# AHupuJR/REFID

Measured on AMD Instinct MI355X. Metric: interpolated frames/sec (train step) GoPro 256x256 11+1, higher is better.
Workload: dtype f32

## Files before the change

refid_amd/csrc/conv_pw.hip:

```cpp
#include "common.h"
#include "conv_args.h"
#include <cstdlib>

namespace {

typedef unsigned int u32x4 __attribute__((ext_vector_type(4)));
typedef __bf16 bf16x8 __attribute__((ext_vector_type(8)));
constexpr int KC = 8;
__device__ constexpr int PW_TA[6] = {0, 1, 0, 2, 0, 1};
__device__ constexpr int PW_TB[6] = {0, 0, 1, 0, 2, 1};

__device__ __forceinline__ void pw_split8(const f32x4& v0, const f32x4& v1, f32x4 (&pl)[3]) {
    bf16x8 p0, p1, p2;
#pragma unroll
    for (int k = 0; k < 8; ++k) {
        const float v = k < 4 ? v0[k] : v1[k - 4];
        const __bf16 h = (__bf16)v;
        p0[k] = h;
        const float r = v - (float)h;
        const __bf16 m = (__bf16)r;
        p1[k] = m;
        p2[k] = (__bf16)(r - (float)m);
    }
    pl[0] = __builtin_bit_cast(f32x4, p0);
    pl[1] = __builtin_bit_cast(f32x4, p1);
    pl[2] = __builtin_bit_cast(f32x4, p2);
}
constexpr int OOB = -1;

__device__ __forceinline__ float gelu_erf(float x) { return 0.5f * x * (1.f + erff(x * 0.70710678118654752440f)); }
__device__ __forceinline__ float gelu_erf_d(float x) {
    const float cdf = 0.5f * (1.f + erff(x * 0.70710678118654752440f));
    const float pdf = 0.39894228040143267794f * __expf(-0.5f * x * x);
    return cdf + x * pdf;
}

template <int NT, int XD, bool EX, bool SIX = false>
__global__ __launch_bounds__(256, (SIX || NT > 2) ? 3 : 4) void conv_pw_kernel(const ConvKArgs a, const PwExtra e) {
    const int lane = threadIdx.x & 63, wave = threadIdx.x >> 6;
    const int li = lane & 31, kh = lane >> 5;
    const long long npix = (long long)a.N * a.H * a.W;
    const long long p0 = ((long long)blockIdx.x * 4 + wave) * 32;
    const long long p = p0 + li;
    const int n0 = blockIdx.y * (32 * NT);

    const long long spanA = a.patchW ? (npix / a.patchW) * (long long)a.patchRow : npix * a.ldA;
    const long long spanB = a.patchW ? spanA - a.patchRow / 2 : npix * (a.inB ? a.ldB : a.ldA);
    const __amdgpu_buffer_rsrc_t rsA = __builtin_amdgcn_make_buffer_rsrc(
        const_cast<float*>(a.inA), 0, (int)min(spanA * 4, 0x7fffffffLL), 0x00020000);
    const __amdgpu_buffer_rsrc_t rsB = __builtin_amdgcn_make_buffer_rsrc(
        const_cast<float*>(a.inB ? a.inB : a.inA), 0, (int)min(spanB * 4, 0x7fffffffLL), 0x00020000);
    const __amdgpu_buffer_rsrc_t rsW = __builtin_amdgcn_make_buffer_rsrc(
        const_cast<float*>(a.w), 0, (int)min((long long)a.nchunks * a.CoutPad * KC * (SIX ? 6 : 4), 0x7fffffffLL), 0x00020000);
    const bool pok = p < npix;
    const long long pA = a.patchW ? (p / a.patchW) * a.patchRow + (p % a.patchW) * a.ldA : p * a.ldA;
    const long long pB = a.patchW ? (p / a.patchW) * a.patchRow + (p % a.patchW) * a.ldB : p * a.ldB;
    const int voA = pok ? (int)(pA * 4) + kh * 16 : OOB;
    const int voB = pok ? (int)(pB * 4) + kh * 16 : OOB;
    int voW[NT];
#pragma unroll
    for (int nt = 0; nt < NT; ++nt) {
        const int row = a.coBase + n0 + nt * 32 + li;
        voW[nt] = (row < a.CoutPad) ? (SIX ? row * 32 + kh * 16 : (row * KC + kh * 4) * 4) : OOB;
    }
    const int wChunk = a.CoutPad * KC * 4;
    const int wPlane = a.CoutPad * 32;

    f32x16 acc[NT];
#pragma unroll
    for (int nt = 0; nt < NT; ++nt)
#pragma unroll
        for (int r = 0; r < 16; ++r) acc[nt][r] = 0.f;

    auto load_x = [&](int ch) -> f32x4 {
        const int c0 = ch * KC;
        const bool fromA = c0 < a.Ca;
        const int soff = (fromA ? c0 : c0 - a.Ca) * 4;
        const int vo = (c0 + kh * 4 < a.Ctot) ? (fromA ? voA : voB) : OOB;
        const u32x4 v = fromA ? __builtin_amdgcn_raw_buffer_load_b128(rsA, vo, soff, 0)
                              : __builtin_amdgcn_raw_buffer_load_b128(rsB, vo, soff, 0);
        return __builtin_bit_cast(f32x4, v);
    };
    auto load_w = [&](int ch, f32x4 (&dst)[NT]) {
#pragma unroll
        for (int nt = 0; nt < NT; ++nt)
            dst[nt] = __builtin_bit_cast(f32x4, __builtin_amdgcn_raw_buffer_load_b128(rsW, voW[nt], ch * wChunk, 0));
    };
    auto load_w6 = [&](int c16, f32x4 (&dst)[3][NT]) {
#pragma unroll
        for (int pl = 0; pl < 3; ++pl)
#pragma unroll
            for (int nt = 0; nt < NT; ++nt)
                dst[pl][nt] = __builtin_bit_cast(f32x4, __builtin_amdgcn_raw_buffer_load_b128(rsW, voW[nt], (c16 * 3 + pl) * wPlane, 0));
    };
    auto mfma6 = [&](const f32x4& x0, const f32x4& x1, const f32x4 (&w6)[3][NT]) {
        f32x4 pl[3];
        pw_split8(x0, x1, pl);
#pragma unroll
        for (int t = 0; t < 6; ++t)
#pragma unroll
            for (int nt = 0; nt < NT; ++nt)
                acc[nt] = __builtin_amdgcn_mfma_f32_32x32x16_bf16(__builtin_bit_cast(bf16x8, w6[PW_TA[t]][nt]),
                                                                  __builtin_bit_cast(bf16x8, pl[PW_TB[t]]), acc[nt], 0, 0, 0);
    };

    f32x4 xr[2 * XD];
    f32x4 wr[SIX ? 1 : 2][NT];
    f32x4 w6[SIX ? 2 : 1][3][NT];
    const int nch = a.nchunks;
    __shared__ float sS[EX ? 128 : 1];
    bool ln_done = false;
    if constexpr (EX) {
        if (e.pool != nullptr) {
            __shared__ float sM[128], sZ[64];
            const int C = e.seC, Ch = C / 2, tid = threadIdx.x;
            const int n = (int)(((long long)blockIdx.x * 128) / e.hw);
            for (int c = tid; c < C; c += 256) {
                const float* pp = e.pool + (long long)n * e.poolParts * C + c;
                float s0 = 0.f;
                for (int r = 0; r < e.poolParts; ++r) s0 += pp[(long long)r * C];
                sM[c] = s0 * e.invHW;
            }
            __syncthreads();
            for (int j = tid; j < Ch; j += 256) {
                float z = e.seB1[j];
                for (int c = 0; c < C; ++c) z += e.seW1[j * C + c] * sM[c];
                sZ[j] = z > 0.f ? z : 0.f;
            }
            __syncthreads();
            for (int c = tid; c < C; c += 256) {
                float v = e.seB2[c];
                for (int j = 0; j < Ch; ++j) v += e.seW2[c * Ch + j] * sZ[j];
                sS[c] = 1.f / (1.f + __expf(-v));
            }
            __syncthreads();
            if (e.seS != nullptr && blockIdx.y == 0 && ((long long)blockIdx.x * 128) % e.hw == 0) {
                for (int c = tid; c < C; c += 256) { e.seM[n * C + c] = sM[c]; e.seS[n * C + c] = sS[c]; }
                for (int j = tid; j < Ch; j += 256) e.seZ1[n * Ch + j] = sZ[j];
            }
        }
        if (e.lnG != nullptr) {
#pragma unroll
            for (int j = 0; j < 2 * XD; ++j) xr[j] = (j < nch) ? load_x(j) : f32x4{0.f, 0.f, 0.f, 0.f};
            if constexpr (SIX) load_w6(0, w6[0]);
            else load_w(0, wr[0]);
            float s1 = 0.f;
#pragma unroll
            for (int j = 0; j < 2 * XD; ++j) s1 += (xr[j][0] + xr[j][1]) + (xr[j][2] + xr[j][3]);
            s1 += __shfl_xor(s1, 32, 64);
            const float mu = s1 / (float)a.Ctot;
            float s2 = 0.f;
#pragma unroll
            for (int j = 0; j < 2 * XD; ++j)
                if (j < nch) {
#pragma unroll
                    for (int k = 0; k < 4; ++k) { const float d = xr[j][k] - mu; s2 += d * d; }
                }
            s2 += __shfl_xor(s2, 32, 64);
            const float rstd = 1.f / sqrtf(s2 / (float)a.Ctot + e.lnEps);
#pragma unroll
            for (int j = 0; j < 2 * XD; ++j)
                if (j < nch) {
                    const int c = j * KC + kh * 4;
                    const f32x4 gv = *reinterpret_cast<const f32x4*>(e.lnG + c);
                    const f32x4 bv = *reinterpret_cast<const f32x4*>(e.lnB + c);
#pragma unroll
                    for (int k = 0; k < 4; ++k) xr[j][k] = (xr[j][k] - mu) * rstd * gv[k] + bv[k];
                    if (e.lnOut != nullptr && blockIdx.y == 0 && pok)
                        *reinterpret_cast<f32x4*>(e.lnOut + p * e.ldLn + c) = xr[j];
                }
            if constexpr (SIX) {
#pragma unroll
                for (int j = 0; j < 2 * XD; j += 2)
                    if (j < nch) {
                        if (j + 2 < nch) load_w6(j / 2 + 1, w6[(j / 2 + 1) & 1]);
                        mfma6(xr[j], xr[j + 1], w6[(j / 2) & 1]);
                    }
            } else {
#pragma unroll
                for (int j = 0; j < 2 * XD; ++j)
                    if (j < nch) {
                        if (j + 1 < nch) load_w(j + 1, wr[(j + 1) & 1]);
#pragma unroll
                        for (int kk = 0; kk < 4; ++kk)
#pragma unroll
                            for (int nt = 0; nt < NT; ++nt)
                                acc[nt] = __builtin_amdgcn_mfma_f32_32x32x2f32(wr[j & 1][nt][kk], xr[j][kk], acc[nt], 0, 0, 0);
                    }
            }
            ln_done = true;
        }
    }
    if (!ln_done) {
#pragma unroll
        for (int j = 0; j < XD; ++j)
            if (j < nch) xr[j] = load_x(j);
        if constexpr (SIX) load_w6(0, w6[0]);
        else load_w(0, wr[0]);
        for (int c0 = 0; c0 < nch; c0 += 2 * XD) {
#pragma unroll
            for (int j = 0; j < 2 * XD; ++j) {
                const int c = c0 + j;
                if (c < nch) {
                    if constexpr (SIX) {
                        if ((j & 1) == 0 && c + 2 < nch) load_w6(c / 2 + 1, w6[(j / 2 + 1) & 1]);
                    } else {
                        if (c + 1 < nch) load_w(c + 1, wr[(j + 1) & 1]);
                    }
                    if (c + XD < nch) xr[(j + XD) % (2 * XD)] = load_x(c + XD);
                    if constexpr (EX) {
                        if (e.pool != nullptr) {
                            const int k0 = c * KC + kh * 4;
                            const f32x4 sv = *reinterpret_cast<const f32x4*>(&sS[k0 % e.seC]);
                            xr[j] *= sv;
                            if (e.xsOut != nullptr && blockIdx.y == 0 && pok)
                                *reinterpret_cast<f32x4*>(e.xsOut + p * e.ldXs + k0) = xr[j];
                        }
                    }
                    if constexpr (SIX) {
                        if (j & 1) mfma6(xr[j - 1], xr[j], w6[(j / 2) & 1]);
                    } else {
#pragma unroll
                        for (int kk = 0; kk < 4; ++kk)
#pragma unroll
                            for (int nt = 0; nt < NT; ++nt)
                                acc[nt] = __builtin_amdgcn_mfma_f32_32x32x2f32(wr[j & 1][nt][kk], xr[j][kk], acc[nt], 0, 0, 0);
                    }
                }
            }
        }
    }

    if (a.vecOK) {
        constexpr int HN = (NT > 2) ? 2 : NT;
        constexpr int PITCH = 8 * HN + 1;
        __shared__ f32x4 sT[4][32 * PITCH];
        f32x4* t = sT[wave];
#pragma unroll
        for (int h0 = 0; h0 < NT; h0 += HN) {
            if (h0) __syncthreads();
#pragma unroll
            for (int nt = 0; nt < HN; ++nt)
#pragma unroll
                for (int g = 0; g < 4; ++g) {
                    f32x4 v;
#pragma unroll
                    for (int k = 0; k < 4; ++k) v[k] = acc[h0 + nt][4 * g + k];
                    t[li * PITCH + nt * 8 + 2 * g + kh] = v;
                }
            __syncthreads();
#pragma unroll
            for (int it = 0; it < 4 * HN; ++it) {
                const int f = it * 64 + lane;
                const int px = f / (8 * HN), c4 = f % (8 * HN);
                const long long pp = p0 + px;
                const int j0 = n0 + h0 * 32 + c4 * 4;
                if (pp >= npix || j0 >= a.Cout) continue;
                f32x4 v = t[px * PITCH + c4];
                if (a.shuffle) {
                    const int Co1 = a.Cout >> 2;
                    const unsigned qd = (unsigned)j0 / (unsigned)Co1, ch = (unsigned)j0 - qd * Co1;
                    const unsigned up = (unsigned)pp, row = up / (unsigned)a.W, x = up - row * a.W;
                    const long long op = (long long)(2 * row + (qd >> 1)) * (2 * a.W) + 2 * x + (qd & 1);
                    if (a.bias) v += *reinterpret_cast<const f32x4*>(a.bias + ch);
                    lrelu4(v, a.slopePre, a.slopePre != 1.f);
                    if (a.res) v += *reinterpret_cast<const f32x4*>(a.res + op * a.ldR + ch);
                    lrelu4(v, a.slopePost, a.slopePost != 1.f);
                    *reinterpret_cast<f32x4*>(a.out + op * a.ldO + ch) = v;
                    continue;
                }
                if (a.bias) v += *reinterpret_cast<const f32x4*>(a.bias + a.coBase + j0);
                lrelu4(v, a.slopePre, a.slopePre != 1.f);
                if (a.res) v += *reinterpret_cast<const f32x4*>(a.res + pp * a.ldR + j0);
                if constexpr (EX) {
                    if (e.res2) v += *reinterpret_cast<const f32x4*>(e.res2 + pp * e.ldR2 + j0);
                }
                lrelu4(v, a.slopePost, a.slopePost != 1.f);
                if (a.mask) {
                    const f32x4 mv = *reinterpret_cast<const f32x4*>(a.mask + pp * a.ldM + j0);
                    if (a.maskMode == 1) {
#pragma unroll
                        for (int k = 0; k < 4; ++k) v[k] *= gelu_erf_d(mv[k]);
                    } else {
#pragma unroll
                        for (int k = 0; k < 4; ++k) v[k] *= (mv[k] > 0.f) ? 1.f : a.slopeMask;
                    }
                }
                *reinterpret_cast<f32x4*>(a.out + pp * a.ldO + j0) = v;
                if (a.out2)
                    *reinterpret_cast<f32x4*>(a.out2 + pp * a.ldO2 + j0) = v + *reinterpret_cast<const f32x4*>(a.add2 + pp * a.ldA2 + j0);
                if constexpr (EX) {
                    if (e.out2) {
                        f32x4 gl;
#pragma unroll
                        for (int k = 0; k < 4; ++k) gl[k] = gelu_erf(v[k]);
                        *reinterpret_cast<f32x4*>(e.out2 + pp * e.ldO2 + j0) = gl;
                    }
                }
            }
        }
        return;
    }
    if (!pok) return;
#pragma unroll
    for (int nt = 0; nt < NT; ++nt) {
#pragma unroll
        for (int g = 0; g < 4; ++g) {
            const int j0 = n0 + nt * 32 + 8 * g + 4 * kh;
#pragma unroll
            for (int k = 0; k < 4; ++k) {
                if (j0 + k >= a.Cout) break;
                float tv = acc[nt][4 * g + k] + (a.bias ? a.bias[a.coBase + j0 + k] : 0.f);
                tv = lrelu(tv, a.slopePre);
                if (a.res) tv += a.res[p * a.ldR + j0 + k];
                tv = lrelu(tv, a.slopePost);
                if (a.mask) tv *= a.maskMode == 1 ? gelu_erf_d(a.mask[p * a.ldM + j0 + k]) : ((a.mask[p * a.ldM + j0 + k] > 0.f) ? 1.f : a.slopeMask);
                a.out[p * a.ldO + j0 + k] = tv;
            }
        }
    }
}

}

int refid_launch_pointwise(const ConvKArgs& ka, hipStream_t st, const PwExtra* ex, int terms) {
    ConvKArgs a = ka;
    a.nchunks = cdiv(a.Ctot, KC);
    const long long npix = (long long)a.N * a.H * a.W;
    const int nb = (int)((npix + 127) / 128);
    const bool six = terms == 6;
    REFID_CHECK(!a.shuffle || (a.vecOK && ex == nullptr && terms == 0 && a.mask == nullptr && a.Cout > 32 && (a.Cout / 4) % 4 == 0 &&
                               npix < 0x7fffffffLL),
                "conv2d: ConvTranspose2d on the pointwise tile needs 16-byte aligned tensors, fp32 products, no mask / fusions and "
                "at least 16 output channels");
    REFID_CHECK(a.out2 == nullptr || (a.vecOK && ex == nullptr), "conv2d: the pointwise tile's second output needs 16-byte aligned tensors and no fusions");
    REFID_CHECK(!a.patchW || (terms == 0 && ex == nullptr && a.inB != nullptr), "conv2d: the patch form of the pointwise tile has fp32 products, no fusions");
    REFID_CHECK(terms == 0 || terms == 6, "conv2d: the pointwise tile has fp32 products (0) or six bf16 products (6), got %d", terms);
    REFID_CHECK(!six || (a.Ctot % 16 == 0 && (a.inB == nullptr || a.Ca % 16 == 0) && a.Cout > 32),
                "conv2d: the six-product pointwise tile needs channel counts that are multiples of 16 and more than 32 outputs");
    if (ex != nullptr) {
        REFID_CHECK(a.vecOK && a.Cout > 32, "conv2d: pointwise fusions need 16-byte aligned tensors and more than 32 outputs");
        REFID_CHECK(!ex->lnG || (a.inB == nullptr && a.Ctot % 8 == 0 && a.Ctot <= 64 && ex->lnB),
                    "conv2d: the LayerNorm prologue needs one source of at most 64 channels (got %d)", a.Ctot);
        REFID_CHECK(!ex->pool || (ex->hw > 0 && ex->hw % 128 == 0 && ex->seC >= 8 && ex->seC <= 128 && ex->seC % 8 == 0 &&
                                  a.Ctot % ex->seC == 0 && ex->poolParts > 0 && ex->seW1 && ex->seB1 && ex->seW2 && ex->seB2 &&
                                  (!ex->seS || (ex->seM && ex->seZ1)) && !ex->lnG),
                    "conv2d: bad squeeze-excite fusion arguments (pixels per sample must be a multiple of 128)");
        if (six) hipLaunchKernelGGL((conv_pw_kernel<2, 4, true, true>), dim3(nb, cdiv(a.Cout, 64)), dim3(256), 0, st, a, *ex);
        else hipLaunchKernelGGL((conv_pw_kernel<2, 4, true>), dim3(nb, cdiv(a.Cout, 64)), dim3(256), 0, st, a, *ex);
        REFID_LAUNCH_CHECK("conv_pw/fused");
        return 0;
    }
    const PwExtra none;
    if (six) hipLaunchKernelGGL((conv_pw_kernel<2, 4, false, true>), dim3(nb, cdiv(a.Cout, 64)), dim3(256), 0, st, a, none);
    else if (a.Cout <= 32) hipLaunchKernelGGL((conv_pw_kernel<1, 8, false>), dim3(nb, 1), dim3(256), 0, st, a, none);
    else {
        static const bool nt4 = []() { const char* e = getenv("REFID_PW_NT4"); return e && e[0] == '1'; }();
        if (nt4 && a.Cout % 128 == 0)
            hipLaunchKernelGGL((conv_pw_kernel<4, 4, false>), dim3(nb, a.Cout / 128), dim3(256), 0, st, a, none);
        else
            hipLaunchKernelGGL((conv_pw_kernel<2, 4, false>), dim3(nb, cdiv(a.Cout, 64)), dim3(256), 0, st, a, none);
    }
    REFID_LAUNCH_CHECK("conv_pw");
    return 0;
}
```

Before: 526.9.

## Software-pipeline pointwise conv main loop and epilogue with buffer loads

Adds a fast main-loop path for channel counts divisible by the unroll group. It uses a deeper weight register ring (for NT==1) and prefetches activations XD chunks ahead, with sched barriers and out-of-bounds buffer loads replacing bounds checks. The LayerNorm prologue gets a fully unrolled specialization with buffer stores, and the SE scaling is folded into the fast loop. The vectorized epilogue now prefetches residual, mask and second-residual tiles through buffer resources ahead of use, and has a dedicated pixel-shuffle path. The aim is to hide global memory latency behind MFMA work and epilogue math, at the cost of more registers and more code complexity.

```diff
diff --git a/refid_amd/csrc/conv_pw.hip b/refid_amd/csrc/conv_pw.hip
--- a/refid_amd/csrc/conv_pw.hip
+++ b/refid_amd/csrc/conv_pw.hip
@@ -1,6 +1,7 @@
 #include "common.h"
 #include "conv_args.h"
 #include <cstdlib>
+#include <type_traits>
 
 namespace {
 
@@ -40,7 +41,7 @@
     const int lane = threadIdx.x & 63, wave = threadIdx.x >> 6;
     const int li = lane & 31, kh = lane >> 5;
     const long long npix = (long long)a.N * a.H * a.W;
-    const long long p0 = ((long long)blockIdx.x * 4 + wave) * 32;
+    const long long p0 = ((long long)blockIdx.x * 4 + __builtin_amdgcn_readfirstlane(wave)) * 32;
     const long long p = p0 + li;
     const int n0 = blockIdx.y * (32 * NT);
 
@@ -86,12 +87,28 @@
         for (int nt = 0; nt < NT; ++nt)
             dst[nt] = __builtin_bit_cast(f32x4, __builtin_amdgcn_raw_buffer_load_b128(rsW, voW[nt], ch * wChunk, 0));
     };
+    auto load_w_sel = [&](int ch, f32x4 (&dst)[NT]) {
+        const bool ok = ch < a.nchunks;
+        const int so = ok ? ch * wChunk : 0;
+#pragma unroll
+        for (int nt = 0; nt < NT; ++nt)
+            dst[nt] = __builtin_bit_cast(f32x4, __builtin_amdgcn_raw_buffer_load_b128(rsW, ok ? voW[nt] : OOB, so, 0));
+    };
     auto load_w6 = [&](int c16, f32x4 (&dst)[3][NT]) {
 #pragma unroll
         for (int pl = 0; pl < 3; ++pl)
 #pragma unroll
             for (int nt = 0; nt < NT; ++nt)
                 dst[pl][nt] = __builtin_bit_cast(f32x4, __builtin_amdgcn_raw_buffer_load_b128(rsW, voW[nt], (c16 * 3 + pl) * wPlane, 0));
+    };
+    auto load_w6_sel = [&](int c16, f32x4 (&dst)[3][NT]) {
+        const bool ok = 2 * c16 < a.nchunks;
+#pragma unroll
+        for (int pl = 0; pl < 3; ++pl)
+#pragma unroll
+            for (int nt = 0; nt < NT; ++nt)
+                dst[pl][nt] = __builtin_bit_cast(f32x4, __builtin_amdgcn_raw_buffer_load_b128(rsW, ok ? voW[nt] : OOB,
+                                                                                              ok ? (c16 * 3 + pl) * wPlane : 0, 0));
     };
     auto mfma6 = [&](const f32x4& x0, const f32x4& x1, const f32x4 (&w6)[3][NT]) {
         f32x4 pl[3];
@@ -104,8 +121,10 @@
                                                                   __builtin_bit_cast(bf16x8, pl[PW_TB[t]]), acc[nt], 0, 0, 0);
     };
 
+    constexpr int WD = (NT == 1) ? 3 : 1;
+    static_assert((2 * XD) % (WD + 1) == 0, "the weight ring must divide the unrolled group");
     f32x4 xr[2 * XD];
-    f32x4 wr[SIX ? 1 : 2][NT];
+    f32x4 wr[SIX ? 1 : WD + 1][NT];
     f32x4 w6[SIX ? 2 : 1][3][NT];
     const int nch = a.nchunks;
     __shared__ float sS[EX ? 128 : 1];
@@ -140,58 +159,136 @@
             }
         }
         if (e.lnG != nullptr) {
-#pragma unroll
-            for (int j = 0; j < 2 * XD; ++j) xr[j] = (j < nch) ? load_x(j) : f32x4{0.f, 0.f, 0.f, 0.f};
+            const __amdgpu_buffer_rsrc_t rsLn = __builtin_amdgcn_make_buffer_rsrc(
+                e.lnOut + p0 * e.ldLn, 0, (e.lnOut != nullptr && blockIdx.y == 0) ? 0x7fffffff : 0, 0x00020000);
+            auto ln_body = [&](auto full_tag) {
+                constexpr bool FULL = decltype(full_tag)::value;
+#pragma unroll
+                for (int j = 0; j < 2 * XD; ++j) xr[j] = (FULL || j < nch) ? load_x(j) : f32x4{0.f, 0.f, 0.f, 0.f};
+                if constexpr (SIX) load_w6(0, w6[0]);
+                else load_w(0, wr[0]);
+                float s1 = 0.f;
+#pragma unroll
+                for (int j = 0; j < 2 * XD; ++j) s1 += (xr[j][0] + xr[j][1]) + (xr[j][2] + xr[j][3]);
+                s1 += __shfl_xor(s1, 32, 64);
+                const float mu = s1 / (float)a.Ctot;
+                float s2 = 0.f;
+#pragma unroll
+                for (int j = 0; j < 2 * XD; ++j)
+                    if (FULL || j < nch) {
+#pragma unroll
+                        for (int k = 0; k < 4; ++k) { const float d = xr[j][k] - mu; s2 += d * d; }
+                    }
+                s2 += __shfl_xor(s2, 32, 64);
+                const float rstd = 1.f / sqrtf(s2 / (float)a.Ctot + e.lnEps);
+#pragma unroll
+                for (int j = 0; j < 2 * XD; ++j)
+                    if (FULL || j < nch) {
+                        const int c = j * KC + kh * 4;
+                        const f32x4 gv = *reinterpret_cast<const f32x4*>(e.lnG + c);
+                        const f32x4 bv = *reinterpret_cast<const f32x4*>(e.lnB + c);
+#pragma unroll
+                        for (int k = 0; k < 4; ++k) xr[j][k] = (xr[j][k] - mu) * rstd * gv[k] + bv[k];
+                        if constexpr (FULL)
+                            __builtin_amdgcn_raw_buffer_store_b128(__builtin_bit_cast(u32x4, xr[j]), rsLn,
+                                                                   pok ? (li * e.ldLn + c) * 4 : OOB, 0, 0);
+                        else if (e.lnOut != nullptr && blockIdx.y == 0 && pok)
+                            *reinterpret_cast<f32x4*>(e.lnOut + p * e.ldLn + c) = xr[j];
+                    }
+                if constexpr (SIX) {
+#pragma unroll
+                    for (int j = 0; j < 2 * XD; j += 2)
+                        if (FULL || j < nch) {
+                            if constexpr (FULL) {
+                                if (j + 2 < 2 * XD) load_w6(j / 2 + 1, w6[(j / 2 + 1) & 1]);
+                                __builtin_amdgcn_sched_barrier(0);
+                            } else {
+                                if (j + 2 < nch) load_w6(j / 2 + 1, w6[(j / 2 + 1) & 1]);
+                            }
+                            mfma6(xr[j], xr[j + 1], w6[(j / 2) & 1]);
+                        }
+                } else {
+#pragma unroll
+                    for (int j = 0; j < 2 * XD; ++j)
+                        if (FULL || j < nch) {
+                            if constexpr (FULL) {
+                                if (j + 1 < 2 * XD) load_w(j + 1, wr[(j + 1) & 1]);
+                                __builtin_amdgcn_sched_barrier(0);
+                            } else {
+                                if (j + 1 < nch) load_w(j + 1, wr[(j + 1) & 1]);
+                            }
+#pragma unroll
+                            for (int kk = 0; kk < 4; ++kk)
+#pragma unroll
+                                for (int nt = 0; nt < NT; ++nt)
+                                    acc[nt] = __builtin_amdgcn_mfma_f32_32x32x2f32(wr[j & 1][nt][kk], xr[j][kk], acc[nt], 0, 0, 0);
+                        }
+                }
+            };
+            if (nch == 2 * XD) ln_body(std::true_type{});
+            else ln_body(std::false_type{});
+            ln_done = true;
+        }
+    }
+    if (!ln_done && nch % (2 * XD) == 0) {
+        auto k_fast = [&](auto se_tag) {
+            constexpr bool SE = decltype(se_tag)::value;
+            __amdgpu_buffer_rsrc_t rsXs = rsA;
+            if constexpr (SE)
+                rsXs = __builtin_amdgcn_make_buffer_rsrc(e.xsOut + p0 * e.ldXs, 0,
+                                                         (e.xsOut != nullptr && blockIdx.y == 0) ? 0x7fffffff : 0, 0x00020000);
             if constexpr (SIX) load_w6(0, w6[0]);
-            else load_w(0, wr[0]);
-            float s1 = 0.f;
-#pragma unroll
-            for (int j = 0; j < 2 * XD; ++j) s1 += (xr[j][0] + xr[j][1]) + (xr[j][2] + xr[j][3]);
-            s1 += __shfl_xor(s1, 32, 64);
-            const float mu = s1 / (float)a.Ctot;
-            float s2 = 0.f;
-#pragma unroll
-            for (int j = 0; j < 2 * XD; ++j)
-                if (j < nch) {
-#pragma unroll
-                    for (int k = 0; k < 4; ++k) { const float d = xr[j][k] - mu; s2 += d * d; }
-                }
-            s2 += __shfl_xor(s2, 32, 64);
-            const float rstd = 1.f / sqrtf(s2 / (float)a.Ctot + e.lnEps);
-#pragma unroll
-            for (int j = 0; j < 2 * XD; ++j)
-                if (j < nch) {
-                    const int c = j * KC + kh * 4;
-                    const f32x4 gv = *reinterpret_cast<const f32x4*>(e.lnG + c);
-                    const f32x4 bv = *reinterpret_cast<const f32x4*>(e.lnB + c);
-#pragma unroll
-                    for (int k = 0; k < 4; ++k) xr[j][k] = (xr[j][k] - mu) * rstd * gv[k] + bv[k];
-                    if (e.lnOut != nullptr && blockIdx.y == 0 && pok)
-                        *reinterpret_cast<f32x4*>(e.lnOut + p * e.ldLn + c) = xr[j];
-                }
-            if constexpr (SIX) {
-#pragma unroll
-                for (int j = 0; j < 2 * XD; j += 2)
-                    if (j < nch) {
-                        if (j + 2 < nch) load_w6(j / 2 + 1, w6[(j / 2 + 1) & 1]);
-                        mfma6(xr[j], xr[j + 1], w6[(j / 2) & 1]);
-                    }
-            } else {
-#pragma unroll
-                for (int j = 0; j < 2 * XD; ++j)
-                    if (j < nch) {
-                        if (j + 1 < nch) load_w(j + 1, wr[(j + 1) & 1]);
+            else {
+#pragma unroll
+                for (int d = 0; d < WD; ++d) load_w(d, wr[d]);
+            }
+            __builtin_amdgcn_sched_barrier(0);
+#pragma unroll
+            for (int j = 0; j < XD; ++j) {
+                xr[j] = load_x(j);
+                __builtin_amdgcn_sched_barrier(0);
+            }
+            for (int c0 = 0; c0 < nch; c0 += 2 * XD) {
+#pragma unroll
+                for (int j = 0; j < 2 * XD; ++j) {
+                    const int c = c0 + j;
+                    if constexpr (SIX) {
+                        if ((j & 1) == 0) {
+                            if (j + 2 < 2 * XD) load_w6(c / 2 + 1, w6[(j / 2 + 1) & 1]);
+                            else load_w6_sel(c / 2 + 1, w6[(j / 2 + 1) & 1]);
+                        }
+                    } else {
+                        if (j + WD < 2 * XD) load_w(c + WD, wr[(j + WD) % (WD + 1)]);
+                        else load_w_sel(c + WD, wr[(j + WD) % (WD + 1)]);
+                    }
+                    xr[(j + XD) % (2 * XD)] = load_x(c + XD);
+                    __builtin_amdgcn_sched_barrier(0);
+                    if constexpr (SE) {
+                        const int k0 = c * KC + kh * 4;
+                        const f32x4 sv = *reinterpret_cast<const f32x4*>(&sS[k0 % e.seC]);
+                        xr[j] *= sv;
+                        __builtin_amdgcn_raw_buffer_store_b128(__builtin_bit_cast(u32x4, xr[j]), rsXs,
+                                                               pok ? (li * e.ldXs + k0) * 4 : OOB, 0, 0);
+                    }
+                    if constexpr (SIX) {
+                        if (j & 1) mfma6(xr[j - 1], xr[j], w6[(j / 2) & 1]);
+                    } else {
 #pragma unroll
                         for (int kk = 0; kk < 4; ++kk)
 #pragma unroll
                             for (int nt = 0; nt < NT; ++nt)
-                                acc[nt] = __builtin_amdgcn_mfma_f32_32x32x2f32(wr[j & 1][nt][kk], xr[j][kk], acc[nt], 0, 0, 0);
-                    }
-            }
-            ln_done = true;
-        }
-    }
-    if (!ln_done) {
+                                acc[nt] = __builtin_amdgcn_mfma_f32_32x32x2f32(wr[j % (WD + 1)][nt][kk], xr[j][kk], acc[nt], 0, 0, 0);
+                    }
+                }
+            }
+        };
+        bool se = false;
+        if constexpr (EX) se = e.pool != nullptr;
+        if constexpr (EX) {
+            if (se) k_fast(std::true_type{});
+        }
+        if (!se) k_fast(std::false_type{});
+    } else if (!ln_done) {
 #pragma unroll
         for (int j = 0; j < XD; ++j)
             if (j < nch) xr[j] = load_x(j);
@@ -234,10 +331,99 @@
     if (a.vecOK) {
         constexpr int HN = (NT > 2) ? 2 : NT;
         constexpr int PITCH = 8 * HN + 1;
+        constexpr int NI = 4 * HN, PD = NT > 2 ? NI / 4 : NI / 2;
+        constexpr int PXI = 64 / (8 * HN);
         __shared__ f32x4 sT[4][32 * PITCH];
         f32x4* t = sT[wave];
+        const int c4 = lane % (8 * HN), pxl = lane / (8 * HN);
+        const int nvalid = (int)max(min(npix - p0, 32LL), 0LL);
+        constexpr int REC = 0x7fffffff, FL = 0x00020000;
+        auto u4 = [](const f32x4& v) { return __builtin_bit_cast(u32x4, v); };
+        auto ld4 = [](__amdgpu_buffer_rsrc_t rs, int vo, int so) {
+            return __builtin_bit_cast(f32x4, __builtin_amdgcn_raw_buffer_load_b128(rs, vo, so, 0));
+        };
+        if (!EX && a.shuffle) {
+            const int Co1 = a.Cout >> 2;
+            const unsigned row0 = (unsigned)p0 / (unsigned)a.W;
+            const long long opb = (long long)(2 * row0) * (2 * a.W);
+            const __amdgpu_buffer_rsrc_t rsBias = __builtin_amdgcn_make_buffer_rsrc(const_cast<float*>(a.bias), 0, a.bias ? REC : 0, FL);
+            const __amdgpu_buffer_rsrc_t rsRes = __builtin_amdgcn_make_buffer_rsrc(const_cast<float*>(a.res) + opb * a.ldR, 0, a.res ? REC : 0, FL);
+            const __amdgpu_buffer_rsrc_t rsOut = __builtin_amdgcn_make_buffer_rsrc(a.out + opb * a.ldO, 0, REC, FL);
+#pragma unroll
+            for (int h0 = 0; h0 < NT; h0 += HN) {
+                const int j0 = n0 + h0 * 32 + c4 * 4;
+                const unsigned qd = (unsigned)j0 / (unsigned)Co1, ch = (unsigned)j0 - qd * Co1;
+                const bool cok = j0 < a.Cout;
+                int dop[NI];
+#pragma unroll
+                for (int it = 0; it < NI; ++it) {
+                    const long long pp = p0 + it * PXI + pxl;
+                    const unsigned up = (unsigned)pp, row = up / (unsigned)a.W, x = up - row * a.W;
+                    dop[it] = (cok & (it * PXI + pxl < nvalid)) ? (int)(2 * (row - row0) + (qd >> 1)) * (2 * a.W) + (int)(2 * x + (qd & 1)) : -1;
+                }
+                auto vo = [&](int it, int ld) { return dop[it] >= 0 ? (dop[it] * ld + (int)ch) * 4 : OOB; };
+                f32x4 pres[NI];
+                const f32x4 bv = ld4(rsBias, cok ? (int)ch * 4 : OOB, 0);
+#pragma unroll
+                for (int i = 0; i < PD; ++i) pres[i] = ld4(rsRes, vo(i, a.ldR), 0);
+                __builtin_amdgcn_sched_barrier(0);
+                if (h0) __syncthreads();
+#pragma unroll
+                for (int nt = 0; nt < HN; ++nt)
+#pragma unroll
+                    for (int g = 0; g < 4; ++g) {
+                        f32x4 v;
+#pragma unroll
+                        for (int k = 0; k < 4; ++k) v[k] = acc[h0 + nt][4 * g + k];
+                        t[li * PITCH + nt * 8 + 2 * g + kh] = v;
+                    }
+                __syncthreads();
+#pragma unroll
+                for (int it = 0; it < NI; ++it) {
+                    if (it + PD < NI) {
+                        pres[it + PD] = ld4(rsRes, vo(it + PD, a.ldR), 0);
+                        __builtin_amdgcn_sched_barrier(0);
+                    }
+                    f32x4 v = t[(it * PXI + pxl) * PITCH + c4];
+                    if (a.bias) v += bv;
+                    lrelu4(v, a.slopePre, a.slopePre != 1.f);
+                    if (a.res) v += pres[it];
+                    lrelu4(v, a.slopePost, a.slopePost != 1.f);
+                    __builtin_amdgcn_raw_buffer_store_b128(u4(v), rsOut, vo(it, a.ldO), 0, 0);
+                }
+            }
+            return;
+        }
+        const __amdgpu_buffer_rsrc_t rsBias = __builtin_amdgcn_make_buffer_rsrc(const_cast<float*>(a.bias) + a.coBase + n0, 0, a.bias ? REC : 0, FL);
+        const __amdgpu_buffer_rsrc_t rsRes = __builtin_amdgcn_make_buffer_rsrc(const_cast<float*>(a.res) + p0 * a.ldR + n0, 0, a.res ? REC : 0, FL);
+        const __amdgpu_buffer_rsrc_t rsMask = __builtin_amdgcn_make_buffer_rsrc(const_cast<float*>(a.mask) + p0 * a.ldM + n0, 0, a.mask ? REC : 0, FL);
+        const float* s3p = EX ? e.res2 : a.add2;
+        const int ldS3 = EX ? e.ldR2 : a.ldA2;
+        float* o2p = EX ? e.out2 : a.out2;
+        const int ldP2 = EX ? e.ldO2 : a.ldO2;
+        const bool has3 = EX ? e.res2 != nullptr : a.out2 != nullptr;
+        const __amdgpu_buffer_rsrc_t rsS3 = __builtin_amdgcn_make_buffer_rsrc(const_cast<float*>(s3p) + p0 * ldS3 + n0, 0, has3 ? REC : 0, FL);
+        const __amdgpu_buffer_rsrc_t rsOut = __builtin_amdgcn_make_buffer_rsrc(a.out + p0 * a.ldO + n0, 0, REC, FL);
+        const __amdgpu_buffer_rsrc_t rsOut2 = __builtin_amdgcn_make_buffer_rsrc(o2p + p0 * ldP2 + n0, 0, o2p ? REC : 0, FL);
 #pragma unroll
         for (int h0 = 0; h0 < NT; h0 += HN) {
+            const bool cok = n0 + h0 * 32 + c4 * 4 < a.Cout;
+            constexpr int so = 0;
+            const int hb = h0 * 32 * 4;
+            auto vo = [&](int it, int ld) {
+                const int px = it * PXI + pxl;
+                return (cok & (px < nvalid)) ? (px * ld + c4 * 4) * 4 + hb : OOB;
+            };
+            f32x4 pres[NI], pmask[NI], ps3[NI];
+            auto request = [&](int it) {
+                pres[it] = ld4(rsRes, vo(it, a.ldR), so);
+                ps3[it] = ld4(rsS3, vo(it, ldS3), so);
+                pmask[it] = ld4(rsMask, vo(it, a.ldM), so);
+            };
+            const f32x4 bv = ld4(rsBias, cok ? c4 * 16 + hb : OOB, so);
+#pragma unroll
+            for (int i = 0; i < PD; ++i) request(i);
+            __builtin_amdgcn_sched_barrier(0);
             if (h0) __syncthreads();
 #pragma unroll
             for (int nt = 0; nt < HN; ++nt)
@@ -250,34 +436,21 @@
                 }
             __syncthreads();
 #pragma unroll
-            for (int it = 0; it < 4 * HN; ++it) {
-                const int f = it * 64 + lane;
-                const int px = f / (8 * HN), c4 = f % (8 * HN);
-                const long long pp = p0 + px;
-                const int j0 = n0 + h0 * 32 + c4 * 4;
-                if (pp >= npix || j0 >= a.Cout) continue;
-                f32x4 v = t[px * PITCH + c4];
-                if (a.shuffle) {
-                    const int Co1 = a.Cout >> 2;
-                    const unsigned qd = (unsigned)j0 / (unsigned)Co1, ch = (unsigned)j0 - qd * Co1;
-                    const unsigned up = (unsigned)pp, row = up / (unsigned)a.W, x = up - row * a.W;
-                    const long long op = (long long)(2 * row + (qd >> 1)) * (2 * a.W) + 2 * x + (qd & 1);
-                    if (a.bias) v += *reinterpret_cast<const f32x4*>(a.bias + ch);
-                    lrelu4(v, a.slopePre, a.slopePre != 1.f);
-                    if (a.res) v += *reinterpret_cast<const f32x4*>(a.res + op * a.ldR + ch);
-                    lrelu4(v, a.slopePost, a.slopePost != 1.f);
-                    *reinterpret_cast<f32x4*>(a.out + op * a.ldO + ch) = v;
-                    continue;
-                }
-                if (a.bias) v += *reinterpret_cast<const f32x4*>(a.bias + a.coBase + j0);
+            for (int it = 0; it < NI; ++it) {
+                if (it + PD < NI) {
+                    request(it + PD);
+                    __builtin_amdgcn_sched_barrier(0);
+                }
+                f32x4 v = t[(it * PXI + pxl) * PITCH + c4];
+                if (a.bias) v += bv;
                 lrelu4(v, a.slopePre, a.slopePre != 1.f);
-                if (a.res) v += *reinterpret_cast<const f32x4*>(a.res + pp * a.ldR + j0);
+                if (a.res) v += pres[it];
                 if constexpr (EX) {
-                    if (e.res2) v += *reinterpret_cast<const f32x4*>(e.res2 + pp * e.ldR2 + j0);
+                    if (e.res2) v += ps3[it];
                 }
                 lrelu4(v, a.slopePost, a.slopePost != 1.f);
                 if (a.mask) {
-                    const f32x4 mv = *reinterpret_cast<const f32x4*>(a.mask + pp * a.ldM + j0);
+                    const f32x4 mv = pmask[it];
                     if (a.maskMode == 1) {
 #pragma unroll
                         for (int k = 0; k < 4; ++k) v[k] *= gelu_erf_d(mv[k]);
@@ -286,16 +459,17 @@
                         for (int k = 0; k < 4; ++k) v[k] *= (mv[k] > 0.f) ? 1.f : a.slopeMask;
                     }
                 }
-                *reinterpret_cast<f32x4*>(a.out + pp * a.ldO + j0) = v;
-                if (a.out2)
-                    *reinterpret_cast<f32x4*>(a.out2 + pp * a.ldO2 + j0) = v + *reinterpret_cast<const f32x4*>(a.add2 + pp * a.ldA2 + j0);
+                __builtin_amdgcn_raw_buffer_store_b128(u4(v), rsOut, vo(it, a.ldO), so, 0);
                 if constexpr (EX) {
                     if (e.out2) {
                         f32x4 gl;
 #pragma unroll
                         for (int k = 0; k < 4; ++k) gl[k] = gelu_erf(v[k]);
-                        *reinterpret_cast<f32x4*>(e.out2 + pp * e.ldO2 + j0) = gl;
-                    }
+                        __builtin_amdgcn_raw_buffer_store_b128(u4(gl), rsOut2, vo(it, ldP2), so, 0);
+                    }
+                } else {
+                    if (a.out2)
+                        __builtin_amdgcn_raw_buffer_store_b128(u4(v + ps3[it]), rsOut2, vo(it, ldP2), so, 0);
                 }
             }
         }
```

Result: no change. 531.9, median of 6 (+1.0%).
